# uzh-rpg/dagr

Measured on NVIDIA H100. Metric: Mevents/sec, higher is better.
Workload: dtype f32

## Files before the change

### dagr_b200/csrc/build_l1.cu

```cuda
#include "common.cuh"

#define BL_THREADS 160
#define BL_CAP 2048
#define BL_CAP_LEAN 1536
#define BL_THREADS_BIG 512
#define BL_CAP_BIG 12288
#define BL_NB 8

struct BLTile {
    int X0, Y0, TW, TH;
    int run_start[3], run_off[3], run_len[3];
    int smin, smax;
    int unsorted;
    int maxidx;
};

__host__ __device__ __forceinline__ size_t bl_acc_offset(const dagr_geom_t &g, int cap, int threads)
{
    const size_t TW = g.CW + 2 * g.r, TH = g.CH + 2 * g.r, TP = TW * TH;
    const size_t o = (size_t)cap * 12 + TP * 4 + (TW + TH) * 4 + TP * BL_NB * 2 + (size_t)g.ncell * 4 + (size_t)threads * 2 + (TW + TH);
    return (o + 15) / 16 * 16;
}
static size_t bl_smem_bytes(const dagr_geom_t *g, int cap, int threads)
{
    const size_t TW = g->CW + 2 * g->r, TH = g->CH + 2 * g->r;
    return bl_acc_offset(*g, cap, threads) + (size_t)(DAGR_ELL - 1) * threads * 4 + (size_t)BL_NB * (TW + TH) * 4 + 16;
}

#define BL_R1 96

template <bool STAGED, int THREADS>
__device__ __forceinline__ void bl_probe(const dagr_geom_t &g, int64_t N, int p, bool active, const int2 me, int eb, int tidx0,
                                         int c_end, const uint32_t *s_pbin, const uint16_t *s_rng, const short *s_sp2,
                                         const int2 *s_ti, const int2 *__restrict__ ti, uint32_t *s_acc,
                                         int32_t *__restrict__ nbr, uint16_t *__restrict__ off, int &n_out)
{
    const int kmax = g.K - 1;
    int n = active ? 0 : kmax;
    for (int c0 = 0; c0 < c_end; c0 += 4) {
        if (__all_sync(0xffffffffu, n >= kmax)) break;
        uint32_t rg[4]; int pix[4];
#pragma unroll
        for (int u = 0; u < 4; u++) {
            const int c = min(c0 + u, g.ncell - 1);
            pix[u] = tidx0 + s_sp2[c];
        }
#pragma unroll
        for (int u = 0; u < 4; u++) rg[u] = s_rng[pix[u] * BL_NB + eb];
#pragma unroll
        for (int u = 0; u < 4; u++) {
            const int c = c0 + u;
            const int lo = rg[u] & 0xff, hi = rg[u] >> 8;
            const int cnt = (c < c_end && n < kmax) ? hi - lo : 0;
            if (!__any_sync(0xffffffffu, cnt > 0)) continue;
            const int base = (int)(s_pbin[pix[u]] >> 8);
            const int vmax = __reduce_max_sync(0xffffffffu, cnt);
            for (int k = 0; k < vmax; k++) {
                if (k < cnt && n < kmax) {
                    const int j = base + hi - 1 - k;
                    const int2 o = STAGED ? s_ti[j] : __ldg(ti + j);
                    if (o.y < me.y && me.x - o.x <= g.dt_us) {
                        if (STAGED) s_acc[n * THREADS + threadIdx.x] = ((uint32_t)j << 10) | (uint32_t)c;
                        else { nbr[(int64_t)n * N + p] = j; off[(int64_t)n * N + p] = (uint16_t)c; }
                        n++;
                    }
                }
            }
        }
    }
    n_out = active ? n : 0;
}


#ifndef BL_SHARED_ADDR
#define BL_SHARED_ADDR 1
#endif
__device__ __forceinline__ uint32_t bl_sa(const void *p) { return (uint32_t)__cvta_generic_to_shared(p); }
__device__ __forceinline__ uint32_t bl_lds32(uint32_t a) { uint32_t v; asm volatile("ld.shared.u32 %0, [%1];" : "=r"(v) : "r"(a) : "memory"); return v; }
__device__ __forceinline__ uint32_t bl_lds16(uint32_t a) { uint32_t v; asm volatile("{ .reg .u16 t; ld.shared.u16 t, [%1]; cvt.u32.u16 %0, t; }" : "=r"(v) : "r"(a) : "memory"); return v; }
__device__ __forceinline__ int bl_lds16s(uint32_t a) { int v; asm volatile("{ .reg .s16 t; ld.shared.s16 t, [%1]; cvt.s32.s16 %0, t; }" : "=r"(v) : "r"(a) : "memory"); return v; }
__device__ __forceinline__ int2 bl_lds64(uint32_t a) { int2 v; asm volatile("ld.shared.v2.s32 {%0, %1}, [%2];" : "=r"(v.x), "=r"(v.y) : "r"(a) : "memory"); return v; }
#ifndef BL_FAST_TABLES
#define BL_FAST_TABLES 1
#endif
__device__ __forceinline__ int bl_div(int t, int d, float inv)
{
#if BL_FAST_TABLES
    if ((unsigned)t >= (1u << 24)) return t / d;
    int q = (int)((float)t * inv);
    const int r = t - q * d;
    if (r < 0) q--; else if (r >= d) q++;
    return q;
#else
    (void)inv;
    return t / d;
#endif
}
__device__ __forceinline__ void bl_sts32(uint32_t a, uint32_t v) { asm volatile("st.shared.u32 [%0], %1;" :: "r"(a), "r"(v) : "memory"); }

template <bool STAGED, int THREADS>
__device__ __forceinline__ void bl_probe_rings(const dagr_geom_t &g, int64_t N, int p, bool active, const int2 me, int eb, int tx0, int ty0,
                                               int TW, int TH, const uint32_t *s_pbin, const uint16_t *s_rng, const uint32_t *s_occ_r,
                                               const uint32_t *s_occ_c, const short *s_sp2, const int2 *s_ti, const int2 *__restrict__ ti, uint32_t *s_acc,
                                               int32_t *__restrict__ nbr, uint16_t *__restrict__ off, int &n_out)
{
    const int kmax = g.K - 1;
    int n = active ? 0 : kmax;
    const uint32_t *occr = s_occ_r + eb * TH, *occc = s_occ_c + eb * TW;
    constexpr bool SA = STAGED && BL_SHARED_ADDR;
    const uint32_t a_rng = bl_sa(s_rng) + 2u * (uint32_t)eb, a_pbin = bl_sa(s_pbin), a_ti = bl_sa(s_ti), a_sp2 = bl_sa(s_sp2);
    const uint32_t a_acc = bl_sa(s_acc) + 4u * threadIdx.x;
    const int dt_us = g.dt_us;
    auto visit = [&](int pix, int c) {
        const uint32_t rg = SA ? bl_lds16(a_rng + (uint32_t)pix * (2u * BL_NB)) : (uint32_t)s_rng[pix * BL_NB + eb];
        const int lo = rg & 0xff, hi = rg >> 8;
        const int base = (int)((SA ? bl_lds32(a_pbin + 4u * (uint32_t)pix) : s_pbin[pix]) >> 8);
        for (int j = base + hi - 1; j >= base + lo && n < kmax; j--) {
            const int2 o = SA ? bl_lds64(a_ti + 8u * (uint32_t)j) : (STAGED ? s_ti[j] : __ldg(ti + j));
            if (o.y < me.y && me.x - o.x <= dt_us) {
                if (SA) bl_sts32(a_acc + (uint32_t)n * (4u * THREADS), ((uint32_t)j << 10) | (uint32_t)c);
                else if (STAGED) s_acc[n * THREADS + threadIdx.x] = ((uint32_t)j << 10) | (uint32_t)c;
                else { nbr[(int64_t)n * N + p] = j; off[(int64_t)n * N + p] = (uint16_t)c; }
                n++;
            }
        }
    };
    if (n < kmax && ((occr[ty0] >> tx0) & 1u)) visit(ty0 * TW + tx0, 0);
    const int tidx0 = ty0 * TW + tx0;
    for (int d = 1; d <= g.r; d++) {
        if (__all_sync(0xffffffffu, n >= kmax)) break;
        const int l2 = 2 * d;
        const uint32_t fm = (l2 >= 32) ? 0xffffffffu : ((1u << l2) - 1u);
        const int cbase = (l2 - 1) * (l2 - 1);
        uint32_t lo = 0, hi = 0;
        if (n < kmax) {
            const uint32_t leg0 = (occc[tx0 + d] >> (ty0 - d + 1)) & fm;
            const uint32_t leg1 = __brev((occr[ty0 + d] >> (tx0 - d)) & fm) >> (32 - l2);
            const uint32_t leg2 = __brev((occc[tx0 - d] >> (ty0 - d)) & fm) >> (32 - l2);
            const uint32_t leg3 = (occr[ty0 - d] >> (tx0 - d + 1)) & fm;
            const unsigned long long m = (unsigned long long)leg0 | ((unsigned long long)leg1 << l2) |
                                         ((unsigned long long)leg2 << (2 * l2)) | ((unsigned long long)leg3 << (3 * l2));
            lo = (uint32_t)m; hi = (uint32_t)(m >> 32);
        }
        while (lo | hi) {
            int i;
            if (lo) { i = __ffs((int)lo) - 1; lo &= lo - 1; }
            else    { i = 32 + __ffs((int)hi) - 1; hi &= hi - 1; }
            visit(tidx0 + (SA ? bl_lds16s(a_sp2 + 2u * (uint32_t)(cbase + i)) : (int)s_sp2[cbase + i]), cbase + i);
            if (n >= kmax) { lo = 0; hi = 0; }
        }
    }
    n_out = active ? n : 0;
}

template <bool STAGED, int THREADS>
__device__ __forceinline__ int bl_probe_coop(const dagr_geom_t &g, int64_t N, int p, const int2 me, int eb, int tidx0, int c_begin,
                                             int n, const uint32_t *s_pbin, const uint16_t *s_rng, const short *s_sp2,
                                             const int2 *s_ti, const int2 *__restrict__ ti, uint32_t *s_acc, int owner,
                                             int32_t *__restrict__ nbr, uint16_t *__restrict__ off)
{
    const int kmax = g.K - 1;
    const int lane = threadIdx.x & 31;
    for (int c0 = c_begin; c0 < g.ncell && n < kmax; c0 += 32) {
        const int c = c0 + lane;
        int cnt = 0, base = 0, hi = 0, acc = 0;
        if (c < g.ncell) {
            const int pix = tidx0 + s_sp2[c];
            const uint32_t rg = s_rng[pix * BL_NB + eb];
            hi = rg >> 8; cnt = hi - (int)(rg & 0xff);
            base = (int)(s_pbin[pix] >> 8);
            for (int k = 0; k < cnt; k++) {
                const int2 o = STAGED ? s_ti[base + hi - 1 - k] : __ldg(ti + base + hi - 1 - k);
                acc += (o.y < me.y && me.x - o.x <= g.dt_us) ? 1 : 0;
            }
        }
        int incl = acc;
#pragma unroll
        for (int d = 1; d < 32; d <<= 1) { const int v = __shfl_up_sync(0xffffffffu, incl, d); if (lane >= d) incl += v; }
        const int tot = __shfl_sync(0xffffffffu, incl, 31);
        if (acc > 0) {
            int slot = n + incl - acc;
            for (int k = 0; k < cnt && slot < kmax; k++) {
                const int j = base + hi - 1 - k;
                const int2 o = STAGED ? s_ti[j] : __ldg(ti + j);
                if (o.y < me.y && me.x - o.x <= g.dt_us) {
                    if (STAGED) s_acc[slot * THREADS + owner] = ((uint32_t)j << 10) | (uint32_t)c;
                    else { nbr[(int64_t)slot * N + p] = j; off[(int64_t)slot * N + p] = (uint16_t)c; }
                    slot++;
                }
            }
        }
        n = min(n + tot, kmax);
    }
    return n;
}

template <int CAP, int THREADS>
__device__ __forceinline__ void bl_voxel(const dagr_geom_t &g, int64_t N, const int32_t *__restrict__ start, const int2 *__restrict__ ti,
                                         const uint32_t *__restrict__ xyb, const float *__restrict__ feat_s, const float *__restrict__ tab,
                                         const dagr_l1a_params_t &P, const int do_conv, const int min_idx, const int32_t *__restrict__ flags,
                                         int32_t *__restrict__ nbr, uint16_t *__restrict__ off, uint32_t *__restrict__ cellmask,
                                         float *__restrict__ xa, const int cell, unsigned char *smem_raw, BLTile &T, uint32_t &s_mask,
                                         int32_t *__restrict__ wl_hdr, int32_t *__restrict__ wl_ids, const int defer)
{
    const int per = g.ny1 * g.nx1;
    const int b = cell / per, rem = cell % per, cy = rem / g.nx1, cx = rem % g.nx1;
    const int p0 = start[(int64_t)cell * g.CP], p1 = start[(int64_t)(cell + 1) * g.CP];
    if (p1 == p0) { if (threadIdx.x == 0 && min_idx <= 0) cellmask[cell] = 0; return; }

    const int TWmax = g.CW + 2 * g.r, THmax = g.CH + 2 * g.r, TPmax = TWmax * THmax;
    int2 *s_ti = (int2 *)smem_raw;
    float *s_feat = (float *)(s_ti + CAP);
    uint16_t *s_rng = (uint16_t *)(s_feat + CAP);
    uint32_t *s_pbin = (uint32_t *)(s_rng + TPmax * BL_NB);
    float *s_posx = (float *)(s_pbin + TPmax);
    float *s_posy = s_posx + TWmax;
    short *s_sp = (short *)(s_posy + THmax);
    short *s_sp2 = s_sp + g.ncell;
    uint16_t *s_order = (uint16_t *)(s_sp2 + g.ncell);
    uint32_t *s_acc = (uint32_t *)(smem_raw + bl_acc_offset(g, CAP, THREADS));
    uint32_t *s_occ_r = s_acc + (DAGR_ELL - 1) * THREADS;
    unsigned char *s_colv = (unsigned char *)(s_order + THREADS);
    unsigned char *s_rowv = s_colv + TWmax;

    const int dtw = max(g.dt_us, 1);
    const float dtw_inv = 1.0f / (float)dtw;
    if (threadIdx.x == 0) {
        const int X0 = g.vx0[cx], X1 = g.vx0[cx + 1], Y0 = g.vy0[cy], Y1 = g.vy0[cy + 1];
        T.X0 = X0 - g.r; T.Y0 = Y0 - g.r; T.TW = X1 - X0 + 2 * g.r; T.TH = Y1 - Y0 + 2 * g.r;
        const int clo = max(cx - 1, 0), chi = min(cx + 1, g.nx1 - 1);
        int o = 0;
        for (int rr = 0; rr < 3; rr++) {
            const int ry = cy - 1 + rr;
            if (ry < 0 || ry >= g.ny1) { T.run_start[rr] = 0; T.run_len[rr] = 0; T.run_off[rr] = o; continue; }
            const int64_t c0 = (int64_t)b * per + ry * g.nx1 + clo, c1 = (int64_t)b * per + ry * g.nx1 + chi + 1;
            const int s = start[c0 * g.CP], e = start[c1 * g.CP];
            T.run_start[rr] = s; T.run_len[rr] = e - s; T.run_off[rr] = o;
            o += e - s;
        }
        T.smin = 0x7fffffff; T.smax = -0x7fffffff; T.unsorted = 0; T.maxidx = -1;
        s_mask = 0;
    }
    __syncthreads();
    const int TW = T.TW, TH = T.TH, TP = TW * TH;
    uint32_t *s_occ_c = s_occ_r + BL_NB * TH;
    const int total = T.run_off[2] + T.run_len[2];
    const bool staged = total <= CAP;
    if (!staged && wl_hdr != nullptr) {
        int slot = 0;
        if (threadIdx.x == 0) slot = atomicAdd(&wl_hdr[0], 1);
        if (defer) { if (threadIdx.x == 0) wl_ids[slot] = cell; return; }
    }
    const int bbase = b * per * g.CP;

    for (int i = threadIdx.x; i < g.ncell; i += blockDim.x) {
        const int dx = g.spiral[2 * i], dy = g.spiral[2 * i + 1];
        s_sp[i] = (short)((dx & 0xff) | (dy << 8));
        s_sp2[i] = (short)(dy * TW + dx);
    }
    for (int i = threadIdx.x; i < TW; i += blockDim.x) {
        const int gx = T.X0 + i;
        const bool in = gx >= 0 && gx < g.W;
        s_posx[i] = in ? g.posx0[gx] : 0.f;
        s_colv[i] = (unsigned char)(in ? (g.xkey[gx] / g.CP - cx + 1) : 1);
    }
    for (int i = threadIdx.x; i < TH; i += blockDim.x) {
        const int gy = T.Y0 + i;
        const bool in = gy >= 0 && gy < g.H;
        s_posy[i] = in ? g.posy0[gy] : 0.f;
        s_rowv[i] = (unsigned char)(in ? (g.ykey[gy] / (g.nx1 * g.CP) - cy + 1) : 1);
    }
    for (int i = threadIdx.x; i < TP; i += blockDim.x) {
        const int ty = i / TW, tx = i % TW;
        const int gx = T.X0 + tx, gy = T.Y0 + ty;
        uint32_t v = 0;
        if (gx >= 0 && gx < g.W && gy >= 0 && gy < g.H) {
            const int ky = g.ykey[gy], kx = g.xkey[gx];
            const int k = bbase + ky + kx;
            const int s = start[k], e = start[k + 1];
            if (e > s) {
                const int lo = max(s, e - g.Q);
                const int rr = ky / (g.nx1 * g.CP) - cy + 1;
                const int pos = staged ? (lo - T.run_start[rr] + T.run_off[rr]) : lo;
                v = ((uint32_t)pos << 8) | (uint32_t)(e - lo);
            }
        }
        s_pbin[i] = v;
    }
    if (staged) {
        for (int rr = 0; rr < 3; rr++) {
            const int s = T.run_start[rr], o = T.run_off[rr], len = T.run_len[rr];
            for (int i = threadIdx.x; i < len; i += blockDim.x) {
                s_ti[o + i] = ti[s + i];
                s_feat[o + i] = feat_s[s + i];
            }
        }
    }
    {
        int mn = 0x7fffffff, mx = -0x7fffffff, mi = -1;
        for (int p = p0 + threadIdx.x; p < p1; p += blockDim.x) {
            const int2 r = ti[p];
            if (r.y < min_idx) continue;
            const int sl = bl_div(r.x, dtw, dtw_inv); mn = min(mn, sl); mx = max(mx, sl); mi = max(mi, r.y);
        }
        mn = __reduce_min_sync(0xffffffffu, mn); mx = __reduce_max_sync(0xffffffffu, mx); mi = __reduce_max_sync(0xffffffffu, mi);
        if ((threadIdx.x & 31) == 0) { atomicMin(&T.smin, mn); atomicMax(&T.smax, mx); atomicMax(&T.maxidx, mi); }
    }
    __syncthreads();
    if (T.maxidx < 0) return;
    const int sbase = T.smin - 1;
    bool bucketed = staged && (T.smax - sbase) < BL_NB && (flags == nullptr || flags[0] == 0);
    const bool use_rings = TW <= 32 && TH <= 32 && g.r <= 8;
    for (int pass = 0; pass < 2; pass++) {
        for (int i = threadIdx.x; i < TP; i += blockDim.x) {
            const uint32_t pb = s_pbin[i];
            const int vis = pb & 0xff, base = pb >> 8;
            unsigned char cum[BL_NB + 1];
#pragma unroll
            for (int q = 0; q <= BL_NB; q++) cum[q] = 0;
            if (bucketed) {
                int prev = 0;
                for (int k = 0; k < vis; k++) {
                    int bk = bl_div(s_ti[base + k].x, dtw, dtw_inv) - sbase;
                    bk = min(max(bk, 0), BL_NB - 1);
                    if (bk < prev) T.unsorted = 1;
                    prev = bk;
#pragma unroll
                    for (int q = 0; q <= BL_NB; q++) cum[q] += (bk < q) ? 1 : 0;
                }
            } else {
#pragma unroll
                for (int q = 1; q <= BL_NB; q++) cum[q] = (unsigned char)vis;
            }
            static_assert(BL_NB == 8, "one uint4 per pixel");
            uint32_t w[4];
#pragma unroll
            for (int e = 0; e < BL_NB; e += 2) {
                const uint32_t r0 = (uint32_t)cum[e > 0 ? e - 1 : 0] | ((uint32_t)cum[e + 1] << 8);
                const uint32_t r1 = (uint32_t)cum[e] | ((uint32_t)cum[e + 2] << 8);
                w[e >> 1] = r0 | (r1 << 16);
            }
            reinterpret_cast<uint4 *>(s_rng)[i] = make_uint4(w[0], w[1], w[2], w[3]);
        }
        __syncthreads();
        if (use_rings) {
            for (int idx = threadIdx.x; idx < BL_NB * (TH + TW); idx += blockDim.x) {
                uint32_t m = 0;
#if BL_FAST_TABLES
                if (idx < BL_NB * TH) {
                    const int e = idx / TH, row = idx % TH;
                    uint32_t a = bl_sa(s_rng) + 2u * (uint32_t)(row * TW * BL_NB + e);
                    for (int x = 0; x < TW; x++, a += 2u * BL_NB) {
                        const uint32_t rg = bl_lds16(a);
                        m |= ((rg >> 8) > (rg & 0xff)) ? (1u << x) : 0u;
                    }
                } else {
                    const int i2 = idx - BL_NB * TH, e = i2 / TW, col = i2 % TW;
                    uint32_t a = bl_sa(s_rng) + 2u * (uint32_t)(col * BL_NB + e);
                    for (int y = 0; y < TH; y++, a += 2u * BL_NB * (uint32_t)TW) {
                        const uint32_t rg = bl_lds16(a);
                        m |= ((rg >> 8) > (rg & 0xff)) ? (1u << y) : 0u;
                    }
                }
#else
                if (idx < BL_NB * TH) {
                    const int e = idx / TH, row = idx % TH;
                    for (int x = 0; x < TW; x++) {
                        const uint32_t rg = s_rng[(row * TW + x) * BL_NB + e];
                        m |= ((rg >> 8) > (rg & 0xff)) ? (1u << x) : 0u;
                    }
                } else {
                    const int i2 = idx - BL_NB * TH, e = i2 / TW, col = i2 % TW;
                    for (int y = 0; y < TH; y++) {
                        const uint32_t rg = s_rng[(y * TW + col) * BL_NB + e];
                        m |= ((rg >> 8) > (rg & 0xff)) ? (1u << y) : 0u;
                    }
                }
#endif
                s_occ_r[idx] = m;
            }
        }
        __syncthreads();
        if (!bucketed || !T.unsorted) break;
        bucketed = false;
    }
    const int nown = p1 - p0;
    const int own_off = staged ? (p0 - T.run_start[1] + T.run_off[1]) : 0;
    uint32_t mloc = 0;
    for (int pb0 = 0; pb0 < nown; pb0 += blockDim.x) {
        const int chunk = min((int)blockDim.x, nown - pb0);
        __syncthreads();
        if (!use_rings && (int)threadIdx.x < chunk) {
            const int myidx = staged ? s_ti[own_off + pb0 + threadIdx.x].y : ti[p0 + pb0 + threadIdx.x].y;
            int rank = 0;
            for (int k = 0; k < chunk; k++) {
                const int oi = staged ? s_ti[own_off + pb0 + k].y : __ldg(&ti[p0 + pb0 + k].y);
                rank += (oi < myidx) ? 1 : 0;
            }
            s_order[rank] = (uint16_t)threadIdx.x;
        }
        __syncthreads();
        const int nw = blockDim.x >> 5;
        const int rank = use_rings ? (int)threadIdx.x : (int)(threadIdx.x & 31) * nw + (int)(threadIdx.x >> 5);
        bool active = rank < chunk;
        const int p = p0 + pb0 + (active ? (use_rings ? rank : (int)s_order[rank]) : 0);
        int x = 0, y = 0;
        int2 me = make_int2(0, 0);
        if (active) {
            const uint32_t w = xyb[p];
            x = w & 0xfff; y = (w >> 12) & 0xfff;
            me = ti[p];
            active = me.y >= min_idx;
        }
        const int tx0 = active ? x - T.X0 : g.r, ty0 = active ? y - T.Y0 : g.r;
        int eb = 0;
        if (bucketed) eb = min(max(bl_div(me.x, dtw, dtw_inv) - sbase, 0), BL_NB - 1);
        int n;
        const int tidx0 = ty0 * TW + tx0;
        if (use_rings) {
            if (staged) bl_probe_rings<true, THREADS>(g, N, p, active, me, eb, tx0, ty0, TW, TH, s_pbin, s_rng, s_occ_r, s_occ_c, s_sp2, s_ti, ti, s_acc, nbr, off, n);
            else        bl_probe_rings<false, THREADS>(g, N, p, active, me, eb, tx0, ty0, TW, TH, s_pbin, s_rng, s_occ_r, s_occ_c, s_sp2, s_ti, ti, s_acc, nbr, off, n);
        } else {
            if (staged) bl_probe<true, THREADS>(g, N, p, active, me, eb, tidx0, BL_R1 < g.ncell ? BL_R1 : g.ncell, s_pbin, s_rng, s_sp2, s_ti, ti, s_acc, nbr, off, n);
            else        bl_probe<false, THREADS>(g, N, p, active, me, eb, tidx0, BL_R1 < g.ncell ? BL_R1 : g.ncell, s_pbin, s_rng, s_sp2, s_ti, ti, s_acc, nbr, off, n);
            if (BL_R1 < g.ncell) {
                unsigned todo = __ballot_sync(0xffffffffu, active && n < g.K - 1);
                while (todo) {
                    const int src = __ffs(todo) - 1;
                    todo &= todo - 1;
                    const int ep = __shfl_sync(0xffffffffu, p, src);
                    const int2 eme = make_int2(__shfl_sync(0xffffffffu, me.x, src), __shfl_sync(0xffffffffu, me.y, src));
                    const int eeb = __shfl_sync(0xffffffffu, eb, src), etidx = __shfl_sync(0xffffffffu, tidx0, src);
                    const int en = __shfl_sync(0xffffffffu, n, src);
                    const int owner = (int)(threadIdx.x & ~31u) + src;
                    const int nn = staged ? bl_probe_coop<true, THREADS>(g, N, ep, eme, eeb, etidx, BL_R1, en, s_pbin, s_rng, s_sp2, s_ti, ti, s_acc, owner, nbr, off)
                                          : bl_probe_coop<false, THREADS>(g, N, ep, eme, eeb, etidx, BL_R1, en, s_pbin, s_rng, s_sp2, s_ti, ti, s_acc, owner, nbr, off);
                    if ((int)(threadIdx.x & 31) == src) n = nn;
                }
                __syncwarp();
            }
        }
        if (active) nbr[(int64_t)(DAGR_ELL - 1) * N + p] = n;
        const float f0 = active ? feat_s[p] : 0.f, f1 = s_posx[tx0], f2 = s_posy[ty0];
        float A[DAGR_KU][3];
        {
#pragma unroll
            for (int u = 0; u < DAGR_KU; u++) { const float t = __ldg(tab + u); A[u][0] = t * f0; A[u][1] = t * f1; A[u][2] = t * f2; }
        }
        const int nmax = __reduce_max_sync(0xffffffffu, n);
        for (int q = 0; q < nmax; q++) {
            if (q < n) {
                int j, c;
                if (staged) { const uint32_t a = s_acc[q * THREADS + threadIdx.x]; j = (int)(a >> 10); c = (int)(a & 0x3ff); }
                else { j = nbr[(int64_t)q * N + p]; c = off[(int64_t)q * N + p]; }
                const int sp = s_sp[c];
                const int tx = tx0 + (int)(signed char)(sp & 0xff), ty = ty0 + (sp >> 8);
                const int rr = s_rowv[ty];
                float e0;
                if (staged) {
                    e0 = s_feat[j];
                    nbr[(int64_t)q * N + p] = j - T.run_off[rr] + T.run_start[rr];
                    off[(int64_t)q * N + p] = (uint16_t)c;
                } else e0 = __ldg(feat_s + j);
                const int dcx = (int)s_colv[tx] - 1, dcy = rr - 1;
                if (dcx | dcy) mloc |= 1u << ((dcy + 1) * 3 + (dcx + 1));
                const float e1 = s_posx[tx], e2 = s_posy[ty];
                const float4 *tr = reinterpret_cast<const float4 *>(tab + c * DAGR_TABW);
                const float4 t0 = __ldg(tr), t1 = __ldg(tr + 1), t2 = __ldg(tr + 2), t3 = __ldg(tr + 3);
                const float t[DAGR_KU] = {t0.x, t0.y, t0.z, t0.w, t1.x, t1.y, t1.z, t1.w, t2.x, t2.y, t2.z, t2.w, t3.x, t3.y, t3.z};
#pragma unroll
                for (int u = 0; u < DAGR_KU; u++) {
                    A[u][0] = fmaf(t[u], e0, A[u][0]);
                    A[u][1] = fmaf(t[u], e1, A[u][1]);
                    A[u][2] = fmaf(t[u], e2, A[u][2]);
                }
            }
        }
        if (!active || !do_conv) continue;
        float o[16];
#pragma unroll
        for (int k = 0; k < 16; k++) o[k] = 0.f;
#pragma unroll
        for (int u = 0; u < DAGR_KU; u++)
#pragma unroll
            for (int ci = 0; ci < 3; ci++)
#pragma unroll
                for (int k = 0; k < 16; k++) o[k] = fmaf(A[u][ci], P.w[u][ci][k], o[k]);
#pragma unroll
        for (int k = 0; k < 16; k++) {
            float r = o[k];
            r = fmaf(f0, P.root[0][k], r);
            r = fmaf(f1, P.root[1][k], r);
            r = fmaf(f2, P.root[2][k], r);
            r = fmaf(r, P.scale[k], P.shift[k]);
            o[k] = P.relu ? fmaxf(r, 0.f) : r;
        }
        const int sw = XA_SWZ(p);
        float4 *dst = reinterpret_cast<float4 *>(xa + (int64_t)p * 8);
        dst[sw] = make_float4(o[0], o[1], o[2], o[3]);
        dst[sw ^ 1] = make_float4(o[4], o[5], o[6], o[7]);
        dst = reinterpret_cast<float4 *>(xa + (N + (int64_t)p) * 8);
        dst[sw] = make_float4(o[8], o[9], o[10], o[11]);
        dst[sw ^ 1] = make_float4(o[12], o[13], o[14], o[15]);
    }
    mloc = __reduce_or_sync(0xffffffffu, mloc);
    if ((threadIdx.x & 31) == 0 && mloc) atomicOr(&s_mask, mloc);
    __syncthreads();
    if (threadIdx.x == 0) cellmask[cell] = (min_idx > 0 ? cellmask[cell] : 0u) | s_mask;
}



template <int CAP, int MIN_CTAS>
__global__ void __launch_bounds__(BL_THREADS, MIN_CTAS)
k_l1_build(const dagr_geom_t g, int64_t N, const int32_t *__restrict__ start, const int2 *__restrict__ ti,
           const uint32_t *__restrict__ xyb, const float *__restrict__ feat_s, const float *__restrict__ tab,
           const __grid_constant__ dagr_l1a_params_t P, const int do_conv, const int min_idx, const int32_t *__restrict__ flags,
           int32_t *__restrict__ nbr, uint16_t *__restrict__ off, uint32_t *__restrict__ cellmask, float *__restrict__ xa,
           int32_t *__restrict__ wl_hdr, int32_t *__restrict__ wl_ids, const int defer)
{
    extern __shared__ __align__(16) unsigned char smem_raw[];
    __shared__ BLTile T;
    __shared__ uint32_t s_mask;
    bl_voxel<CAP, BL_THREADS>(g, N, start, ti, xyb, feat_s, tab, P, do_conv, min_idx, flags, nbr, off, cellmask, xa,
                              (int)blockIdx.x, smem_raw, T, s_mask, wl_hdr, wl_ids, defer);
}

__global__ void __launch_bounds__(BL_THREADS_BIG, 1)
k_l1_build_dense(const dagr_geom_t g, int64_t N, const int32_t *__restrict__ start, const int2 *__restrict__ ti,
                 const uint32_t *__restrict__ xyb, const float *__restrict__ feat_s, const float *__restrict__ tab,
                 const __grid_constant__ dagr_l1a_params_t P, const int do_conv, const int min_idx, const int32_t *__restrict__ flags,
                 int32_t *__restrict__ nbr, uint16_t *__restrict__ off, uint32_t *__restrict__ cellmask, float *__restrict__ xa,
                 int32_t *__restrict__ wl_hdr, const int32_t *__restrict__ wl_ids)
{
    extern __shared__ __align__(16) unsigned char smem_raw[];
    __shared__ BLTile T;
    __shared__ uint32_t s_mask;
    __shared__ int s_next;
    const int count = wl_hdr[0];
    for (;;) {
        __syncthreads();
        if (threadIdx.x == 0) s_next = atomicAdd(&wl_hdr[1], 1);
        __syncthreads();
        const int i = s_next;
        if (i >= count) break;
        bl_voxel<BL_CAP_BIG, BL_THREADS_BIG>(g, N, start, ti, xyb, feat_s, tab, P, do_conv, min_idx, flags, nbr, off, cellmask, xa,
                                             wl_ids[i], smem_raw, T, s_mask, nullptr, nullptr, 0);
    }
}

extern "C" int dagr_l1_build(const dagr_geom_t *g, int64_t N, const int32_t *start, const int32_t *ti,
                             const uint32_t *xyb, const float *feat_s, const float *tab,
                             const dagr_l1a_params_t *p_host, const int32_t *flags, int min_idx, int32_t *nbr, uint16_t *off,
                             uint32_t *cellmask, float *xa, int32_t *wl_hdr, int32_t *wl_ids, int defer, void *stream)
{
    DAGR_CHECK_ARG(g, "null argument");
    static const dagr_l1a_params_t zero_params = {};
    const int do_conv = p_host != nullptr;
    if (!p_host) p_host = &zero_params;
    DAGR_CHECK_ARG(g->K >= 1 && g->K <= DAGR_ELL, "max_neighbors must be in [1,16]");
    DAGR_CHECK_ARG(g->r >= 0 && g->r <= 15 && g->Q <= 255, "radius must be <= 15 px and max_queue_size <= 255");
    DAGR_CHECK_ARG(N < (1ll << 24), "the staged probe packs positions in 24 bits (N < 16.7M per call)");
    const int cells = g->B * g->ny1 * g->nx1;
    const bool deferring = wl_hdr != nullptr && wl_ids != nullptr && defer;
    if (deferring) {
        const size_t smem = bl_smem_bytes(g, BL_CAP, BL_THREADS);
        auto kern = k_l1_build<BL_CAP, 4>;
        DAGR_CUDA(dagr_allow_smem(kern, smem, true));
        kern<<<cells, BL_THREADS, smem, (cudaStream_t)stream>>>(*g, N, start, (const int2 *)ti, xyb, feat_s, tab, *p_host, do_conv, min_idx,
                                                                flags, nbr, off, cellmask, xa, wl_hdr, wl_ids, 1);
    } else {
        const size_t smem = bl_smem_bytes(g, BL_CAP_LEAN, BL_THREADS);
        auto kern = k_l1_build<BL_CAP_LEAN, 5>;
        DAGR_CUDA(dagr_allow_smem(kern, smem, true));
        kern<<<cells, BL_THREADS, smem, (cudaStream_t)stream>>>(*g, N, start, (const int2 *)ti, xyb, feat_s, tab, *p_host, do_conv, min_idx,
                                                                flags, nbr, off, cellmask, xa, wl_hdr, wl_ids, 0);
    }
    DAGR_CHECK_LAUNCH();
    if (deferring) {
        const size_t smem_big = bl_smem_bytes(g, BL_CAP_BIG, BL_THREADS_BIG);
        static int n_sm = 0;
        if (n_sm == 0) {
            int dev = 0;
            DAGR_CUDA(cudaGetDevice(&dev));
            DAGR_CUDA(cudaDeviceGetAttribute(&n_sm, cudaDevAttrMultiProcessorCount, dev));
        }
        DAGR_CUDA(dagr_allow_smem(k_l1_build_dense, smem_big));
        k_l1_build_dense<<<n_sm, BL_THREADS_BIG, smem_big, (cudaStream_t)stream>>>(*g, N, start, (const int2 *)ti, xyb, feat_s, tab,
                                                                                    *p_host, do_conv, min_idx, flags, nbr, off,
                                                                                    cellmask, xa, wl_hdr, wl_ids);
        DAGR_CHECK_LAUNCH();
    }
    return DAGR_OK;
}
```

Before: 528.4.

## Factor spline table into separable shared weights and build ring masks via warp ballots

Replaces the per-offset global spline table lookups (15 floats per edge) with separable x/y weight vectors staged in shared memory and multiplied on the fly. The occupancy ring masks are now built with warp ballots and shared atomics while computing pixel ranges, instead of a separate pass that rescans s_rng. Row/column cell classification uses arithmetic instead of lookup tables, s_order aliases the occupancy buffer to save shared memory, and the edge loop is specialised on staged vs unstaged at compile time. This trades global table bandwidth for extra multiplies and adds complexity and rounding-order differences.

```diff
diff --git a/dagr_b200/csrc/build_l1.cu b/dagr_b200/csrc/build_l1.cu
--- a/dagr_b200/csrc/build_l1.cu
+++ b/dagr_b200/csrc/build_l1.cu
@@ -1,3 +1,4 @@
+#include <type_traits>
 #include "common.cuh"
 
 #define BL_THREADS 160
@@ -12,19 +13,21 @@
     int run_start[3], run_off[3], run_len[3];
     int smin, smax;
     int unsorted;
+    int bucketed;
     int maxidx;
 };
 
-__host__ __device__ __forceinline__ size_t bl_acc_offset(const dagr_geom_t &g, int cap, int threads)
+__host__ __device__ __forceinline__ size_t bl_acc_offset(const dagr_geom_t &g, int cap)
 {
     const size_t TW = g.CW + 2 * g.r, TH = g.CH + 2 * g.r, TP = TW * TH;
-    const size_t o = (size_t)cap * 12 + TP * 4 + (TW + TH) * 4 + TP * BL_NB * 2 + (size_t)g.ncell * 4 + (size_t)threads * 2 + (TW + TH);
+    const size_t o = (size_t)(2 * g.r + 1) * 32 + (size_t)cap * 12 + TP * 4 + (TW + TH) * 4 + TP * BL_NB * 2 + (size_t)g.ncell * 4;
     return (o + 15) / 16 * 16;
 }
 static size_t bl_smem_bytes(const dagr_geom_t *g, int cap, int threads)
 {
     const size_t TW = g->CW + 2 * g->r, TH = g->CH + 2 * g->r;
-    return bl_acc_offset(*g, cap, threads) + (size_t)(DAGR_ELL - 1) * threads * 4 + (size_t)BL_NB * (TW + TH) * 4 + 16;
+    const size_t occ = (size_t)BL_NB * (TW + TH) * 4, order = (size_t)threads * 2;
+    return bl_acc_offset(*g, cap) + (size_t)(DAGR_ELL - 1) * threads * 4 + (occ > order ? occ : order) + 16;
 }
 
 #define BL_R1 96
@@ -197,7 +200,7 @@
 
 template <int CAP, int THREADS>
 __device__ __forceinline__ void bl_voxel(const dagr_geom_t &g, int64_t N, const int32_t *__restrict__ start, const int2 *__restrict__ ti,
-                                         const uint32_t *__restrict__ xyb, const float *__restrict__ feat_s, const float *__restrict__ tab,
+                                         const uint32_t *__restrict__ xyb, const float *__restrict__ feat_s,
                                          const dagr_l1a_params_t &P, const int do_conv, const int min_idx, const int32_t *__restrict__ flags,
                                          int32_t *__restrict__ nbr, uint16_t *__restrict__ off, uint32_t *__restrict__ cellmask,
                                          float *__restrict__ xa, const int cell, unsigned char *smem_raw, BLTile &T, uint32_t &s_mask,
@@ -208,20 +211,21 @@
     const int p0 = start[(int64_t)cell * g.CP], p1 = start[(int64_t)(cell + 1) * g.CP];
     if (p1 == p0) { if (threadIdx.x == 0 && min_idx <= 0) cellmask[cell] = 0; return; }
 
-    const int TWmax = g.CW + 2 * g.r, THmax = g.CH + 2 * g.r, TPmax = TWmax * THmax;
-    int2 *s_ti = (int2 *)smem_raw;
+    const int TWmax = g.CW + 2 * g.r, THmax = g.CH + 2 * g.r, TPmax = TWmax * THmax, R = 2 * g.r + 1;
+    float4 *s_wy = (float4 *)smem_raw;
+    float *s_wx = (float *)(s_wy + R);
+    float *s_wy4 = s_wx + 3 * R;
+    int2 *s_ti = (int2 *)(s_wy4 + R);
     float *s_feat = (float *)(s_ti + CAP);
     uint16_t *s_rng = (uint16_t *)(s_feat + CAP);
     uint32_t *s_pbin = (uint32_t *)(s_rng + TPmax * BL_NB);
     float *s_posx = (float *)(s_pbin + TPmax);
     float *s_posy = s_posx + TWmax;
-    short *s_sp = (short *)(s_posy + THmax);
-    short *s_sp2 = s_sp + g.ncell;
-    uint16_t *s_order = (uint16_t *)(s_sp2 + g.ncell);
-    uint32_t *s_acc = (uint32_t *)(smem_raw + bl_acc_offset(g, CAP, THREADS));
+    uint16_t *s_sp = (uint16_t *)(s_posy + THmax);
+    short *s_sp2 = (short *)(s_sp + g.ncell);
+    uint32_t *s_acc = (uint32_t *)(smem_raw + bl_acc_offset(g, CAP));
     uint32_t *s_occ_r = s_acc + (DAGR_ELL - 1) * THREADS;
-    unsigned char *s_colv = (unsigned char *)(s_order + THREADS);
-    unsigned char *s_rowv = s_colv + TWmax;
+    uint16_t *s_order = (uint16_t *)s_occ_r;
 
     const int dtw = max(g.dt_us, 1);
     const float dtw_inv = 1.0f / (float)dtw;
@@ -243,6 +247,7 @@
     }
     __syncthreads();
     const int TW = T.TW, TH = T.TH, TP = TW * TH;
+    const bool use_rings = TW <= 32 && TH <= 32 && g.r <= 8;
     uint32_t *s_occ_c = s_occ_r + BL_NB * TH;
     const int total = T.run_off[2] + T.run_len[2];
     const bool staged = total <= CAP;
@@ -255,20 +260,22 @@
 
     for (int i = threadIdx.x; i < g.ncell; i += blockDim.x) {
         const int dx = g.spiral[2 * i], dy = g.spiral[2 * i + 1];
-        s_sp[i] = (short)((dx & 0xff) | (dy << 8));
+        s_sp[i] = (uint16_t)((dx + g.r) | ((dy + g.r) << 5));
         s_sp2[i] = (short)(dy * TW + dx);
+    }
+    for (int i = threadIdx.x; i < R; i += blockDim.x) {
+        const float4 tx = __ldg(reinterpret_cast<const float4 *>(g.tabx) + i);
+        s_wx[i] = tx.x; s_wx[R + i] = tx.y; s_wx[2 * R + i] = tx.z;
+        s_wy[i] = __ldg(reinterpret_cast<const float4 *>(g.taby) + 2 * i);
+        s_wy4[i] = __ldg(g.taby + 8 * i + 4);
     }
     for (int i = threadIdx.x; i < TW; i += blockDim.x) {
         const int gx = T.X0 + i;
-        const bool in = gx >= 0 && gx < g.W;
-        s_posx[i] = in ? g.posx0[gx] : 0.f;
-        s_colv[i] = (unsigned char)(in ? (g.xkey[gx] / g.CP - cx + 1) : 1);
+        s_posx[i] = (gx >= 0 && gx < g.W) ? g.posx0[gx] : 0.f;
     }
     for (int i = threadIdx.x; i < TH; i += blockDim.x) {
         const int gy = T.Y0 + i;
-        const bool in = gy >= 0 && gy < g.H;
-        s_posy[i] = in ? g.posy0[gy] : 0.f;
-        s_rowv[i] = (unsigned char)(in ? (g.ykey[gy] / (g.nx1 * g.CP) - cy + 1) : 1);
+        s_posy[i] = (gy >= 0 && gy < g.H) ? g.posy0[gy] : 0.f;
     }
     for (int i = threadIdx.x; i < TP; i += blockDim.x) {
         const int ty = i / TW, tx = i % TW;
@@ -296,6 +303,8 @@
             }
         }
     }
+    if (use_rings)
+        for (int i = threadIdx.x; i < BL_NB * TW; i += blockDim.x) s_occ_c[i] = 0;
     {
         int mn = 0x7fffffff, mx = -0x7fffffff, mi = -1;
         for (int p = p0 + threadIdx.x; p < p1; p += blockDim.x) {
@@ -310,91 +319,81 @@
     if (T.maxidx < 0) return;
     const int sbase = T.smin - 1;
     bool bucketed = staged && (T.smax - sbase) < BL_NB && (flags == nullptr || flags[0] == 0);
-    const bool use_rings = TW <= 32 && TH <= 32 && g.r <= 8;
+    auto pixel_ranges = [&](int i) -> uint32_t {
+        const uint32_t pb = s_pbin[i];
+        const int vis = pb & 0xff, base = pb >> 8;
+        unsigned char cum[BL_NB + 1];
+#pragma unroll
+        for (int q = 0; q <= BL_NB; q++) cum[q] = 0;
+        if (bucketed) {
+            int prev = 0;
+            for (int k = 0; k < vis; k++) {
+                int bk = bl_div(s_ti[base + k].x, dtw, dtw_inv) - sbase;
+                bk = min(max(bk, 0), BL_NB - 1);
+                if (bk < prev) T.unsorted = 1;
+                prev = bk;
+#pragma unroll
+                for (int q = 0; q <= BL_NB; q++) cum[q] += (bk < q) ? 1 : 0;
+            }
+        } else {
+#pragma unroll
+            for (int q = 1; q <= BL_NB; q++) cum[q] = (unsigned char)vis;
+        }
+        static_assert(BL_NB == 8, "one uint4 per pixel");
+        uint32_t w[4], occ = 0;
+#pragma unroll
+        for (int e = 0; e < BL_NB; e += 2) {
+            const uint32_t r0 = (uint32_t)cum[e > 0 ? e - 1 : 0] | ((uint32_t)cum[e + 1] << 8);
+            const uint32_t r1 = (uint32_t)cum[e] | ((uint32_t)cum[e + 2] << 8);
+            w[e >> 1] = r0 | (r1 << 16);
+            occ |= (cum[e + 1] > cum[e > 0 ? e - 1 : 0] ? 1u : 0u) << e;
+            occ |= (cum[e + 2] > cum[e] ? 1u : 0u) << (e + 1);
+        }
+        reinterpret_cast<uint4 *>(s_rng)[i] = make_uint4(w[0], w[1], w[2], w[3]);
+        return occ;
+    };
     for (int pass = 0; pass < 2; pass++) {
-        for (int i = threadIdx.x; i < TP; i += blockDim.x) {
-            const uint32_t pb = s_pbin[i];
-            const int vis = pb & 0xff, base = pb >> 8;
-            unsigned char cum[BL_NB + 1];
-#pragma unroll
-            for (int q = 0; q <= BL_NB; q++) cum[q] = 0;
-            if (bucketed) {
-                int prev = 0;
-                for (int k = 0; k < vis; k++) {
-                    int bk = bl_div(s_ti[base + k].x, dtw, dtw_inv) - sbase;
-                    bk = min(max(bk, 0), BL_NB - 1);
-                    if (bk < prev) T.unsorted = 1;
-                    prev = bk;
-#pragma unroll
-                    for (int q = 0; q <= BL_NB; q++) cum[q] += (bk < q) ? 1 : 0;
+        if (use_rings) {
+            const int lane = threadIdx.x & 31;
+            uint32_t colm[BL_NB];
+#pragma unroll
+            for (int e = 0; e < BL_NB; e++) colm[e] = 0;
+            for (int row = threadIdx.x >> 5; row < TH; row += blockDim.x >> 5) {
+                const uint32_t occ = lane < TW ? pixel_ranges(row * TW + lane) : 0u;
+#pragma unroll
+                for (int e = 0; e < BL_NB; e++) {
+                    const uint32_t m = __ballot_sync(0xffffffffu, (occ >> e) & 1u);
+                    if (lane == e) s_occ_r[e * TH + row] = m;
+                    colm[e] |= ((occ >> e) & 1u) << row;
                 }
-            } else {
-#pragma unroll
-                for (int q = 1; q <= BL_NB; q++) cum[q] = (unsigned char)vis;
-            }
-            static_assert(BL_NB == 8, "one uint4 per pixel");
-            uint32_t w[4];
-#pragma unroll
-            for (int e = 0; e < BL_NB; e += 2) {
-                const uint32_t r0 = (uint32_t)cum[e > 0 ? e - 1 : 0] | ((uint32_t)cum[e + 1] << 8);
-                const uint32_t r1 = (uint32_t)cum[e] | ((uint32_t)cum[e + 2] << 8);
-                w[e >> 1] = r0 | (r1 << 16);
-            }
-            reinterpret_cast<uint4 *>(s_rng)[i] = make_uint4(w[0], w[1], w[2], w[3]);
-        }
-        __syncthreads();
-        if (use_rings) {
-            for (int idx = threadIdx.x; idx < BL_NB * (TH + TW); idx += blockDim.x) {
-                uint32_t m = 0;
-#if BL_FAST_TABLES
-                if (idx < BL_NB * TH) {
-                    const int e = idx / TH, row = idx % TH;
-                    uint32_t a = bl_sa(s_rng) + 2u * (uint32_t)(row * TW * BL_NB + e);
-                    for (int x = 0; x < TW; x++, a += 2u * BL_NB) {
-                        const uint32_t rg = bl_lds16(a);
-                        m |= ((rg >> 8) > (rg & 0xff)) ? (1u << x) : 0u;
-                    }
-                } else {
-                    const int i2 = idx - BL_NB * TH, e = i2 / TW, col = i2 % TW;
-                    uint32_t a = bl_sa(s_rng) + 2u * (uint32_t)(col * BL_NB + e);
-                    for (int y = 0; y < TH; y++, a += 2u * BL_NB * (uint32_t)TW) {
-                        const uint32_t rg = bl_lds16(a);
-                        m |= ((rg >> 8) > (rg & 0xff)) ? (1u << y) : 0u;
-                    }
-                }
-#else
-                if (idx < BL_NB * TH) {
-                    const int e = idx / TH, row = idx % TH;
-                    for (int x = 0; x < TW; x++) {
-                        const uint32_t rg = s_rng[(row * TW + x) * BL_NB + e];
-                        m |= ((rg >> 8) > (rg & 0xff)) ? (1u << x) : 0u;
-                    }
-                } else {
-                    const int i2 = idx - BL_NB * TH, e = i2 / TW, col = i2 % TW;
-                    for (int y = 0; y < TH; y++) {
-                        const uint32_t rg = s_rng[(y * TW + col) * BL_NB + e];
-                        m |= ((rg >> 8) > (rg & 0xff)) ? (1u << y) : 0u;
-                    }
-                }
-#endif
-                s_occ_r[idx] = m;
-            }
+            }
+            if (lane < TW) {
+#pragma unroll
+                for (int e = 0; e < BL_NB; e++)
+                    if (colm[e]) atomicOr(&s_occ_c[e * TW + lane], colm[e]);
+            }
+        } else {
+            for (int i = threadIdx.x; i < TP; i += blockDim.x) pixel_ranges(i);
         }
         __syncthreads();
         if (!bucketed || !T.unsorted) break;
         bucketed = false;
-    }
-    const int nown = p1 - p0;
-    const int own_off = staged ? (p0 - T.run_start[1] + T.run_off[1]) : 0;
+        if (use_rings) {
+            for (int i = threadIdx.x; i < BL_NB * TW; i += blockDim.x) s_occ_c[i] = 0;
+            __syncthreads();
+        }
+    }
+    if (threadIdx.x == 0) T.bucketed = bucketed;
     uint32_t mloc = 0;
-    for (int pb0 = 0; pb0 < nown; pb0 += blockDim.x) {
-        const int chunk = min((int)blockDim.x, nown - pb0);
+    for (int pb = p0; pb < p1; pb += blockDim.x) {
+        const int chunk = min((int)blockDim.x, p1 - pb);
         __syncthreads();
         if (!use_rings && (int)threadIdx.x < chunk) {
-            const int myidx = staged ? s_ti[own_off + pb0 + threadIdx.x].y : ti[p0 + pb0 + threadIdx.x].y;
+            const int d = T.run_off[1] - T.run_start[1];
+            const int myidx = staged ? s_ti[d + pb + threadIdx.x].y : ti[pb + threadIdx.x].y;
             int rank = 0;
             for (int k = 0; k < chunk; k++) {
-                const int oi = staged ? s_ti[own_off + pb0 + k].y : __ldg(&ti[p0 + pb0 + k].y);
+                const int oi = staged ? s_ti[d + pb + k].y : __ldg(&ti[pb + k].y);
                 rank += (oi < myidx) ? 1 : 0;
             }
             s_order[rank] = (uint16_t)threadIdx.x;
@@ -403,7 +402,7 @@
         const int nw = blockDim.x >> 5;
         const int rank = use_rings ? (int)threadIdx.x : (int)(threadIdx.x & 31) * nw + (int)(threadIdx.x >> 5);
         bool active = rank < chunk;
-        const int p = p0 + pb0 + (active ? (use_rings ? rank : (int)s_order[rank]) : 0);
+        const int p = pb + (active ? (use_rings ? rank : (int)s_order[rank]) : 0);
         int x = 0, y = 0;
         int2 me = make_int2(0, 0);
         if (active) {
@@ -414,7 +413,7 @@
         }
         const int tx0 = active ? x - T.X0 : g.r, ty0 = active ? y - T.Y0 : g.r;
         int eb = 0;
-        if (bucketed) eb = min(max(bl_div(me.x, dtw, dtw_inv) - sbase, 0), BL_NB - 1);
+        if (T.bucketed) eb = min(max(bl_div(me.x, dtw, dtw_inv) - sbase, 0), BL_NB - 1);
         int n;
         const int tidx0 = ty0 * TW + tx0;
         if (use_rings) {
@@ -444,39 +443,59 @@
         const float f0 = active ? feat_s[p] : 0.f, f1 = s_posx[tx0], f2 = s_posy[ty0];
         float A[DAGR_KU][3];
         {
-#pragma unroll
-            for (int u = 0; u < DAGR_KU; u++) { const float t = __ldg(tab + u); A[u][0] = t * f0; A[u][1] = t * f1; A[u][2] = t * f2; }
-        }
-        const int nmax = __reduce_max_sync(0xffffffffu, n);
-        for (int q = 0; q < nmax; q++) {
-            if (q < n) {
+            const int o = g.r;
+            const float4 wya = s_wy[o];
+            const float wy[5] = {wya.x, wya.y, wya.z, wya.w, s_wy4[o]}, wx[3] = {s_wx[o], s_wx[R + o], s_wx[2 * R + o]};
+#pragma unroll
+            for (int jy = 0; jy < 5; jy++)
+#pragma unroll
+                for (int k = 0; k < 3; k++) {
+                    const float t = __fmul_rn(wy[jy], wx[k]);
+                    A[k + 3 * jy][0] = t * f0; A[k + 3 * jy][1] = t * f1; A[k + 3 * jy][2] = t * f2;
+                }
+        }
+        int txy = (tx0 - g.r) | ((ty0 - g.r) << 16);
+        auto edges = [&](auto staged_c) {
+            constexpr bool ST = decltype(staged_c)::value;
+            for (int q = 0; q < n; q++) {
+                const uint32_t e = (uint32_t)q * (uint32_t)N + (uint32_t)p;
                 int j, c;
-                if (staged) { const uint32_t a = s_acc[q * THREADS + threadIdx.x]; j = (int)(a >> 10); c = (int)(a & 0x3ff); }
-                else { j = nbr[(int64_t)q * N + p]; c = off[(int64_t)q * N + p]; }
-                const int sp = s_sp[c];
-                const int tx = tx0 + (int)(signed char)(sp & 0xff), ty = ty0 + (sp >> 8);
-                const int rr = s_rowv[ty];
+                if (ST) { const uint32_t a = s_acc[q * THREADS + threadIdx.x]; j = (int)(a >> 10); c = (int)(a & 0x3ff); }
+                else { j = nbr[e]; c = off[e]; }
+                const uint32_t sp = s_sp[c];
+                const int dxi = (int)(sp & 31u), dyi = (int)(sp >> 5);
+                const int txy_e = txy + dxi + (dyi << 16);
+                const int tx = txy_e & 0xffff, ty = txy_e >> 16;
+                const int vr = (ty >= g.r) + (ty + g.r >= TH), vc = (tx >= g.r) + (tx + g.r >= TW);
                 float e0;
-                if (staged) {
+                if (ST) {
                     e0 = s_feat[j];
-                    nbr[(int64_t)q * N + p] = j - T.run_off[rr] + T.run_start[rr];
-                    off[(int64_t)q * N + p] = (uint16_t)c;
+                    nbr[e] = j - T.run_off[vr] + T.run_start[vr];
+                    off[e] = (uint16_t)c;
                 } else e0 = __ldg(feat_s + j);
-                const int dcx = (int)s_colv[tx] - 1, dcy = rr - 1;
-                if (dcx | dcy) mloc |= 1u << ((dcy + 1) * 3 + (dcx + 1));
+                mloc |= 1u << (vr * 3 + vc);
                 const float e1 = s_posx[tx], e2 = s_posy[ty];
-                const float4 *tr = reinterpret_cast<const float4 *>(tab + c * DAGR_TABW);
-                const float4 t0 = __ldg(tr), t1 = __ldg(tr + 1), t2 = __ldg(tr + 2), t3 = __ldg(tr + 3);
-                const float t[DAGR_KU] = {t0.x, t0.y, t0.z, t0.w, t1.x, t1.y, t1.z, t1.w, t2.x, t2.y, t2.z, t2.w, t3.x, t3.y, t3.z};
-#pragma unroll
-                for (int u = 0; u < DAGR_KU; u++) {
-                    A[u][0] = fmaf(t[u], e0, A[u][0]);
-                    A[u][1] = fmaf(t[u], e1, A[u][1]);
-                    A[u][2] = fmaf(t[u], e2, A[u][2]);
-                }
-            }
-        }
+                const float4 wya = s_wy[dyi];
+                const float wy[5] = {wya.x, wya.y, wya.z, wya.w, s_wy4[dyi]}, wx[3] = {s_wx[dxi], s_wx[R + dxi], s_wx[2 * R + dxi]};
+#pragma unroll
+                for (int jy = 0; jy < 5; jy++)
+#pragma unroll
+                    for (int k = 0; k < 3; k++) {
+                        const int u = k + 3 * jy;
+                        const float t = __fmul_rn(wy[jy], wx[k]);
+                        A[u][0] = fmaf(t, e0, A[u][0]);
+                        A[u][1] = fmaf(t, e1, A[u][1]);
+                        A[u][2] = fmaf(t, e2, A[u][2]);
+                    }
+            }
+        };
+        if (staged) edges(std::true_type{});
+        else        edges(std::false_type{});
+
         if (!active || !do_conv) continue;
+        int pr = p;
+        asm volatile("" : "+r"(txy), "+r"(pr));
+        const float r0 = __ldg(feat_s + pr), r1 = s_posx[(txy & 0xffff) + g.r], r2 = s_posy[(txy >> 16) + g.r];
         float o[16];
 #pragma unroll
         for (int k = 0; k < 16; k++) o[k] = 0.f;
@@ -489,9 +508,9 @@
 #pragma unroll
         for (int k = 0; k < 16; k++) {
             float r = o[k];
-            r = fmaf(f0, P.root[0][k], r);
-            r = fmaf(f1, P.root[1][k], r);
-            r = fmaf(f2, P.root[2][k], r);
+            r = fmaf(r0, P.root[0][k], r);
+            r = fmaf(r1, P.root[1][k], r);
+            r = fmaf(r2, P.root[2][k], r);
             r = fmaf(r, P.scale[k], P.shift[k]);
             o[k] = P.relu ? fmaxf(r, 0.f) : r;
         }
@@ -503,7 +522,7 @@
         dst[sw] = make_float4(o[8], o[9], o[10], o[11]);
         dst[sw ^ 1] = make_float4(o[12], o[13], o[14], o[15]);
     }
-    mloc = __reduce_or_sync(0xffffffffu, mloc);
+    mloc = __reduce_or_sync(0xffffffffu, mloc) & ~(1u << 4);
     if ((threadIdx.x & 31) == 0 && mloc) atomicOr(&s_mask, mloc);
     __syncthreads();
     if (threadIdx.x == 0) cellmask[cell] = (min_idx > 0 ? cellmask[cell] : 0u) | s_mask;
@@ -514,7 +533,7 @@
 template <int CAP, int MIN_CTAS>
 __global__ void __launch_bounds__(BL_THREADS, MIN_CTAS)
 k_l1_build(const dagr_geom_t g, int64_t N, const int32_t *__restrict__ start, const int2 *__restrict__ ti,
-           const uint32_t *__restrict__ xyb, const float *__restrict__ feat_s, const float *__restrict__ tab,
+           const uint32_t *__restrict__ xyb, const float *__restrict__ feat_s,
            const __grid_constant__ dagr_l1a_params_t P, const int do_conv, const int min_idx, const int32_t *__restrict__ flags,
            int32_t *__restrict__ nbr, uint16_t *__restrict__ off, uint32_t *__restrict__ cellmask, float *__restrict__ xa,
            int32_t *__restrict__ wl_hdr, int32_t *__restrict__ wl_ids, const int defer)
@@ -522,13 +541,13 @@
     extern __shared__ __align__(16) unsigned char smem_raw[];
     __shared__ BLTile T;
     __shared__ uint32_t s_mask;
-    bl_voxel<CAP, BL_THREADS>(g, N, start, ti, xyb, feat_s, tab, P, do_conv, min_idx, flags, nbr, off, cellmask, xa,
+    bl_voxel<CAP, BL_THREADS>(g, N, start, ti, xyb, feat_s, P, do_conv, min_idx, flags, nbr, off, cellmask, xa,
                               (int)blockIdx.x, smem_raw, T, s_mask, wl_hdr, wl_ids, defer);
 }
 
 __global__ void __launch_bounds__(BL_THREADS_BIG, 1)
 k_l1_build_dense(const dagr_geom_t g, int64_t N, const int32_t *__restrict__ start, const int2 *__restrict__ ti,
-                 const uint32_t *__restrict__ xyb, const float *__restrict__ feat_s, const float *__restrict__ tab,
+                 const uint32_t *__restrict__ xyb, const float *__restrict__ feat_s,
                  const __grid_constant__ dagr_l1a_params_t P, const int do_conv, const int min_idx, const int32_t *__restrict__ flags,
                  int32_t *__restrict__ nbr, uint16_t *__restrict__ off, uint32_t *__restrict__ cellmask, float *__restrict__ xa,
                  int32_t *__restrict__ wl_hdr, const int32_t *__restrict__ wl_ids)
@@ -544,7 +563,7 @@
         __syncthreads();
         const int i = s_next;
         if (i >= count) break;
-        bl_voxel<BL_CAP_BIG, BL_THREADS_BIG>(g, N, start, ti, xyb, feat_s, tab, P, do_conv, min_idx, flags, nbr, off, cellmask, xa,
+        bl_voxel<BL_CAP_BIG, BL_THREADS_BIG>(g, N, start, ti, xyb, feat_s, P, do_conv, min_idx, flags, nbr, off, cellmask, xa,
                                              wl_ids[i], smem_raw, T, s_mask, nullptr, nullptr, 0);
     }
 }
@@ -555,6 +574,7 @@
                              uint32_t *cellmask, float *xa, int32_t *wl_hdr, int32_t *wl_ids, int defer, void *stream)
 {
     DAGR_CHECK_ARG(g, "null argument");
+    (void)tab;
     static const dagr_l1a_params_t zero_params = {};
     const int do_conv = p_host != nullptr;
     if (!p_host) p_host = &zero_params;
@@ -567,13 +587,13 @@
         const size_t smem = bl_smem_bytes(g, BL_CAP, BL_THREADS);
         auto kern = k_l1_build<BL_CAP, 4>;
         DAGR_CUDA(dagr_allow_smem(kern, smem, true));
-        kern<<<cells, BL_THREADS, smem, (cudaStream_t)stream>>>(*g, N, start, (const int2 *)ti, xyb, feat_s, tab, *p_host, do_conv, min_idx,
+        kern<<<cells, BL_THREADS, smem, (cudaStream_t)stream>>>(*g, N, start, (const int2 *)ti, xyb, feat_s, *p_host, do_conv, min_idx,
                                                                 flags, nbr, off, cellmask, xa, wl_hdr, wl_ids, 1);
     } else {
         const size_t smem = bl_smem_bytes(g, BL_CAP_LEAN, BL_THREADS);
         auto kern = k_l1_build<BL_CAP_LEAN, 5>;
         DAGR_CUDA(dagr_allow_smem(kern, smem, true));
-        kern<<<cells, BL_THREADS, smem, (cudaStream_t)stream>>>(*g, N, start, (const int2 *)ti, xyb, feat_s, tab, *p_host, do_conv, min_idx,
+        kern<<<cells, BL_THREADS, smem, (cudaStream_t)stream>>>(*g, N, start, (const int2 *)ti, xyb, feat_s, *p_host, do_conv, min_idx,
                                                                 flags, nbr, off, cellmask, xa, wl_hdr, wl_ids, 0);
     }
     DAGR_CHECK_LAUNCH();
@@ -586,7 +606,7 @@
             DAGR_CUDA(cudaDeviceGetAttribute(&n_sm, cudaDevAttrMultiProcessorCount, dev));
         }
         DAGR_CUDA(dagr_allow_smem(k_l1_build_dense, smem_big));
-        k_l1_build_dense<<<n_sm, BL_THREADS_BIG, smem_big, (cudaStream_t)stream>>>(*g, N, start, (const int2 *)ti, xyb, feat_s, tab,
+        k_l1_build_dense<<<n_sm, BL_THREADS_BIG, smem_big, (cudaStream_t)stream>>>(*g, N, start, (const int2 *)ti, xyb, feat_s,
                                                                                     *p_host, do_conv, min_idx, flags, nbr, off,
                                                                                     cellmask, xa, wl_hdr, wl_ids);
         DAGR_CHECK_LAUNCH();
```

Result: faster. 547.2, median of 6 (+3.6%).
